# tkkim-robot/safe_control

Hardware: AMD Instinct MI355X
Metric: QP solves/sec (batched agents) (higher is better)
Workload: dtype f64; 1 GPU; 4096-agent batch DynamicUnicycle2D CBF-QP, 8 obstacles each (BASELINE configs[1]); agents_per_gpu=4096, obstacles=8, storage=f32, arithmetic=f64, launch=hipGraph

## Files before the change

### safe_control_amd/csrc/cbf_qp_kernel.hpp

```cpp
#pragma once
#include <hip/hip_runtime.h>

#include <utility>

#include <cstdlib>

#include "sc_qp2.hpp"
#include "sc_group.hpp"

namespace sc {

#ifndef SC_COOP_MAX_AGENTS
#define SC_COOP_MAX_AGENTS 32768
#endif

static inline long long sc_coop_max_agents() {
    static const long long v = [] { const char* e = getenv("SC_COOP_MAX_AGENTS"); return e ? atoll(e) : (long long)SC_COOP_MAX_AGENTS; }();
    return v;
}
static inline bool sc_two_pass() {
    static const bool v = [] { const char* e = getenv("SC_CBFQP_TWO_PASS"); return !(e && e[0] == '0'); }();
    return v;
}
static inline bool sc_force_lds_kernel() {
    static const bool v = [] { const char* e = getenv("SC_FORCE_LDS_KERNEL"); return e && e[0] == '1'; }();
    return v;
}

using as1_void = const __attribute__((address_space(1))) void;
using as3_void = __attribute__((address_space(3))) void;

template <typename TIO, int MODEL>
struct StateRow { TIO v[MODEL == SC_MODEL_QUAD2D ? 5 : 4]; };

template <typename TIO, int MODEL>
__device__ __forceinline__ StateRow<TIO, MODEL> load_state(const TIO* __restrict__ X, long long agent) {
    StateRow<TIO, MODEL> s;
    if constexpr (MODEL == SC_MODEL_QUAD2D) {
        const TIO* r = X + agent * 6;
#pragma unroll
        for (int i = 0; i < 5; ++i) s.v[i] = r[i];
    } else {
        const TIO* r = X + agent * 4;
#pragma unroll
        for (int i = 0; i < 4; ++i) s.v[i] = r[i];
    }
    return s;
}

template <typename TIO, typename TC, int MODEL>
__device__ __forceinline__ Agent<TC> to_agent(const StateRow<TIO, MODEL>& s) {
    if constexpr (MODEL == SC_MODEL_QUAD2D) return make_agent_m<TC, MODEL>(TC(s.v[0]), TC(s.v[1]), TC(s.v[2]), TC(s.v[3]), TC(s.v[4]));
    else return make_agent_m<TC, MODEL>(TC(s.v[0]), TC(s.v[1]), TC(s.v[2]), TC(s.v[3]));
}

template <typename TIO, typename TC, int MODEL>
__device__ __forceinline__ Agent<TC> load_agent(const TIO* __restrict__ X, long long agent) {
    return to_agent<TIO, TC, MODEL>(load_state<TIO, MODEL>(X, agent));
}

template <typename T>
__device__ __forceinline__ void fetch_arg_now(const T& v) { asm volatile("" ::"s"(v)); }

template <typename TIO> struct vec2;
template <> struct vec2<float> { using type = float2; };
template <> struct vec2<double> { using type = double2; };

__device__ __forceinline__ void wave_dma16(const unsigned char* __restrict__ src, unsigned char* lds,
                                           unsigned bytes, int lane) {
    const unsigned n16 = bytes >> 4;
    for (unsigned base = 0; base < n16; base += 64) {
        const unsigned idx = base + lane;
        if (idx < n16) {
            __builtin_amdgcn_global_load_lds((as1_void*)(src + (size_t)idx * 16),
                                             (as3_void*)(lds + (size_t)base * 16), 16, 0, 0);
        }
    }
}

template <typename TIO> struct vec4io;
template <> struct vec4io<float> { using type = float4; static constexpr int N = 4; };
template <> struct vec4io<double> { using type = double2; static constexpr int N = 2; };

#define SC_STATUS_PENDING (-1)
template <typename TIO, typename TC, int KMAX, int MODEL, int PASS = 0>
__global__ __launch_bounds__(256) void cbfqp_reg_kernel(const TIO* __restrict__ obs, const TIO* __restrict__ X,
                                                        const TIO* __restrict__ u_ref, const int* __restrict__ n_obs,
                                                        const long long B, const int K, const int obs_shared,
                                                        TIO* __restrict__ u_out, int* __restrict__ status_out,
                                                        TIO* __restrict__ h_out, const CbfConsts<TC> k) {
    const long long agent = (long long)blockIdx.x * blockDim.x + threadIdx.x;
    const bool active = agent < B;
    const long long ag_i = active ? agent : 0;
    using V2 = typename vec2<TIO>::type;
    using V4 = typename vec4io<TIO>::type;
    constexpr int VN = vec4io<TIO>::N;
    if constexpr (PASS == 2) {
        const bool pending = active && status_out[ag_i] == SC_STATUS_PENDING;
        if (__builtin_amdgcn_ballot_w64(pending) == 0ull) return;
    }

    TIO flat[KMAX * 7];
    const TIO* src = obs + (obs_shared ? 0 : (size_t)ag_i * K * 7);
    if (K == KMAX && ((KMAX * 7) % VN == 0) && ((reinterpret_cast<uintptr_t>(obs) & 15u) == 0) &&
        ((KMAX * 7 * sizeof(TIO)) % 16 == 0)) {
        const V4* s4 = reinterpret_cast<const V4*>(src);
#pragma unroll
        for (int e = 0; e < KMAX * 7 / VN; ++e) {
            const V4 q = s4[e];
            if constexpr (VN == 4) {
                flat[e * 4 + 0] = q.x; flat[e * 4 + 1] = q.y; flat[e * 4 + 2] = q.z; flat[e * 4 + 3] = q.w;
            } else {
                flat[e * 2 + 0] = q.x; flat[e * 2 + 1] = q.y;
            }
        }
    } else {
#pragma unroll
        for (int r = 0; r < KMAX; ++r) {
#pragma unroll
            for (int f = 0; f < 7; ++f) flat[r * 7 + f] = (r < K) ? src[r * 7 + f] : TIO(0);
        }
    }
    const V2 ur = reinterpret_cast<const V2*>(u_ref)[ag_i];
    const StateRow<TIO, MODEL> xs = load_state<TIO, MODEL>(X, ag_i);
    int nk = K;
    if (n_obs) nk = n_obs[ag_i];
    nk = nk < 0 ? 0 : (nk > K ? K : nk);
    if constexpr (PASS == 1) {
        bool other = false;
#pragma unroll
        for (int r = 0; r < KMAX; ++r) other |= (r < nk) && (flat[r * 7 + 6] != TIO(0));
        if (__builtin_amdgcn_ballot_w64(other && active) != 0ull) {
            if (active) status_out[agent] = SC_STATUS_PENDING;
            return;
        }
    }
    const TC ur0 = TC(ur.x), ur1 = TC(ur.y);
    const Agent<TC> ag = to_agent<TIO, TC, MODEL>(xs);

    TC n0[KMAX], n1[KMAX], c[KMAX];
    TIO hv[KMAX];
    bool bad_obs = false;
    TC poison = TC(0);
#pragma unroll
    for (int r = 0; r < KMAX; ++r) {
        TC o[7];
#pragma unroll
        for (int f = 0; f < 7; ++f) o[f] = TC(flat[r * 7 + f]);
        TC h, a0, a1, cc;
        const bool ok = cbf_row<TC, MODEL, true, PASS == 1>(ag, o, k, a0, a1, cc, h);
        const bool used = r < nk;
        bad_obs |= used && !ok;
        a0 = used ? a0 : TC(0); a1 = used ? a1 : TC(0); cc = used ? cc : TC(0);
        normalise_row(a0, a1, cc, poison);
        n0[r] = a0; n1[r] = a1; c[r] = cc;
        hv[r] = used ? TIO(h) : TIO(0);
    }

    TC u0, u1;
    int st = qp2_solve<TC, KMAX>(n0, n1, c, K, ur0, ur1, poison, k, u0, u1);
    if (bad_obs) st = SC_STATUS_BAD_OBSTACLE;
    if (st != SC_STATUS_OPTIMAL) { u0 = num<TC>::nan(); u1 = num<TC>::nan(); }
    if (active) {
        V2 uo; uo.x = TIO(u0); uo.y = TIO(u1);
        reinterpret_cast<V2*>(u_out)[agent] = uo;
        status_out[agent] = st;
        if (h_out) {
            TIO* hp = h_out + agent * K;
            if (K == KMAX && (KMAX % VN == 0) && ((reinterpret_cast<uintptr_t>(h_out) & 15u) == 0)) {
                V4* h4 = reinterpret_cast<V4*>(hp);
#pragma unroll
                for (int e = 0; e < KMAX / VN; ++e) {
                    V4 q;
                    if constexpr (VN == 4) { q.x = hv[e * 4]; q.y = hv[e * 4 + 1]; q.z = hv[e * 4 + 2]; q.w = hv[e * 4 + 3]; }
                    else { q.x = hv[e * 2]; q.y = hv[e * 2 + 1]; }
                    h4[e] = q;
                }
            } else {
#pragma unroll
                for (int r = 0; r < KMAX; ++r) if (r < K) hp[r] = hv[r];
            }
        }
    }
}

template <typename TIO, typename TC, int G, int MODEL>
#ifndef SC_COOP_WAVES
#define SC_COOP_WAVES 1
#endif
__global__ __launch_bounds__(64 * SC_COOP_WAVES) void cbfqp_coop_kernel(const TIO* __restrict__ obs, const TIO* __restrict__ X,
                                                        const TIO* __restrict__ u_ref, const int* __restrict__ n_obs,
                                                        const long long B, const int K, const int obs_shared,
                                                        TIO* __restrict__ u_out, int* __restrict__ status_out,
                                                        TIO* __restrict__ h_out, const CbfConsts<TC> k) {
#ifdef SC_EXP_EMPTY
    return;
#endif
    constexpr int APW = 64 / G;
    const int lane = threadIdx.x & 63;
    const int sub = lane & (G - 1);
    const long long agent = ((long long)blockIdx.x * SC_COOP_WAVES + (threadIdx.x >> 6)) * APW + lane / G;
    const bool active = agent < B;
    const long long ag_i = active ? agent : 0;
    using V2 = typename vec2<TIO>::type;
#ifdef SC_EXP_ARGS
    if (active && sub == 0)
        status_out[agent] = (int)((reinterpret_cast<uintptr_t>(obs) ^ reinterpret_cast<uintptr_t>(X) ^ reinterpret_cast<uintptr_t>(u_ref) ^
                                   reinterpret_cast<uintptr_t>(n_obs) ^ reinterpret_cast<uintptr_t>(u_out) ^ reinterpret_cast<uintptr_t>(h_out)) >> 4) + K + obs_shared;
    return;
#endif

    TIO orow[7];
    const bool has_row = sub < K;
    const TIO* src = obs + (obs_shared ? 0 : (size_t)ag_i * K * 7) + (has_row ? sub * 7 : 0);
#pragma unroll
    for (int f = 0; f < 7; ++f) orow[f] = src[f];
    const V2 ur = reinterpret_cast<const V2*>(u_ref)[ag_i];
    const StateRow<TIO, MODEL> xs = load_state<TIO, MODEL>(X, ag_i);
    int nk = K;
    if (n_obs) nk = n_obs[ag_i];
    nk = nk < 0 ? 0 : (nk > K ? K : nk);
    fetch_arg_now(status_out); fetch_arg_now(h_out);
    fetch_arg_now(k.R); fetch_arg_now(k.g1); fetch_arg_now(k.g2);
    fetch_arg_now(k.lo0); fetch_arg_now(k.hi0); fetch_arg_now(k.lo1); fetch_arg_now(k.hi1); fetch_arg_now(k.hard);
#ifdef SC_EXP_LOADS
    if (active) {
        if (sub == 0) {
            V2 uo; uo.x = ur.x + xs.v[0] + xs.v[1]; uo.y = ur.y + xs.v[2] + xs.v[3];
            reinterpret_cast<V2*>(u_out)[agent] = uo;
            status_out[agent] = nk;
        }
        if (h_out && has_row) h_out[agent * K + sub] = orow[0] + orow[1] + orow[2] + orow[3] + orow[4] + orow[5] + orow[6];
    }
    return;
#endif
    const TC ur0 = TC(ur.x), ur1 = TC(ur.y);
    const Agent<TC> ag = to_agent<TIO, TC, MODEL>(xs);

    TC o[7];
#pragma unroll
    for (int f = 0; f < 7; ++f) o[f] = TC(orow[f]);
    TC h, a0, a1, cc;
#ifndef SC_EXP_NOROW
    const bool ok = cbf_row<TC, MODEL, false>(ag, o, k, a0, a1, cc, h);
#else
    const bool ok = true; a0 = o[0] - ag.x; a1 = o[1] - ag.y; cc = o[2]; h = o[3];
#endif
    const bool used = sub < nk;
    const bool bad_mine = used && !ok;
    a0 = used ? a0 : TC(0); a1 = used ? a1 : TC(0); cc = used ? cc : TC(0);
    if (active && h_out && has_row) h_out[agent * K + sub] = used ? TIO(h) : TIO(0);
    TC poison = TC(0);
    normalise_row(a0, a1, cc, poison);

    QpState<TC> S;
    qp_begin(S, ur0, ur1, k);
#ifndef SC_EXP_NOWALK
#ifndef SC_COOP_OLD_WALK
    if constexpr (G == 8) coop_solve_all8<TC>(S, K, sub, lane, a0, a1, cc, k);
    else if constexpr (G == 16) coop_solve_all16<TC>(S, K, sub, lane, a0, a1, cc, k);
    else
#endif
    coop_walk_violated<TC, G>(S, K, sub, lane, a0, a1, cc, k);
#endif
    qp_finish_box(S, k);
    TC worst = qp_row_margin(num<TC>::inf(), a0, a1, cc, S.u0, S.u1, poison);
    const bool nan_mine = !(poison == poison);
    worst = nan_mine ? -num<TC>::inf() : worst;
    if constexpr (G == 8) worst = min8_raw(worst);
    else if constexpr (G == 16) worst = min16_raw(worst);
    else worst = group_min<TC, G>(worst);
    const unsigned long long bad_mask = __builtin_amdgcn_ballot_w64(bad_mine);
    const bool bad_any = ((bad_mask >> (lane & ~(G - 1))) & (G == 64 ? ~0ull : ((1ull << G) - 1ull))) != 0ull;
    int st = qp_status(S, worst, TC(0), k);
    if (bad_any) st = SC_STATUS_BAD_OBSTACLE;
    TC u0 = S.u0, u1 = S.u1;
    if (st != SC_STATUS_OPTIMAL) { u0 = num<TC>::nan(); u1 = num<TC>::nan(); }
    if (active) {
        if (sub == 0) {
            V2 uo; uo.x = TIO(u0); uo.y = TIO(u1);
            reinterpret_cast<V2*>(u_out)[agent] = uo;
            status_out[agent] = st;
        }
    }
}

typedef double sc_d8 __attribute__((ext_vector_type(8)));
struct Coop8Consts {
    sc_d8 t0;
    sc_d8 t1;
    sc_d8 k0;
    sc_d8 k1;
    int hard;
    unsigned B;
};

__device__ __forceinline__ void normalise_row_as_generic(double& n0, double& n1, double& c, double& poison) {
    const double nn = __builtin_fma(n1, n1, n0 * n0);
    poison += 0.0 * (nn + c);
    const double inv = nn > 0.0 ? rsqrt_(nn) : 1.0;
    n0 *= inv; n1 *= inv; c *= inv;
}

template <typename TIO, bool FULL, bool HAS_H>
__global__ __launch_bounds__(64) void cbfqp_coop8_du_kernel(const TIO* __restrict__ obs, const TIO* __restrict__ X,
                                                            const TIO* __restrict__ u_ref, TIO* __restrict__ u_out,
                                                            TIO* __restrict__ h_out, int* __restrict__ status_out,
                                                            const Coop8Consts c) {
#ifdef SC_EXP_EMPTY
    return;
#endif
    using TC = double;
    using V2 = typename vec2<TIO>::type;
    const unsigned lane = threadIdx.x;
    const unsigned sub = lane & 7u;
    const unsigned slot = blockIdx.x * 64u + lane;
    const unsigned agent = slot >> 3;
    bool active = true;
    if constexpr (!FULL) active = agent < c.B;
    const unsigned row_i = active ? slot : sub;
    const unsigned ag_i = row_i >> 3;

    struct { TIO v[7]; } orow;
    __builtin_memcpy(&orow, obs + row_i * 7u, sizeof(orow));
    const V2 ur = reinterpret_cast<const V2*>(u_ref)[ag_i];
    const StateRow<TIO, SC_MODEL_DYNAMIC_UNICYCLE2D> xs = load_state<TIO, SC_MODEL_DYNAMIC_UNICYCLE2D>(X, ag_i);
    fetch_arg_now(c.t0); fetch_arg_now(c.t1); fetch_arg_now(c.k0); fetch_arg_now(c.k1); fetch_arg_now(c.hard);

    SinCosTab sc;
    sc.two_over_pi = c.t0[0]; sc.pio2_1 = c.t0[1]; sc.pio2_2 = c.t0[2]; sc.pio2_3 = c.t0[3];
    sc.s[0] = c.t0[4]; sc.s[1] = c.t0[5]; sc.s[2] = c.t0[6]; sc.s[3] = c.t0[7]; sc.s[4] = c.t1[0]; sc.s[5] = c.t1[1];
#pragma unroll
    for (int i = 0; i < 6; ++i) sc.c[i] = c.t1[2 + i];
    CbfConsts<TC> k;
    k.R = c.k0[0]; k.a1 = TC(0); k.a2 = TC(0); k.g1 = c.k0[1]; k.g2 = c.k0[2]; k.inv_dt = c.k0[3]; k.inv_dt2 = c.k0[4];
    k.lo0 = c.k0[5]; k.hi0 = c.k0[6]; k.lo1 = c.k0[7]; k.hi1 = c.k1[0]; k.inv_Lr = TC(0); k.inv_mass = TC(1); k.hard = c.hard;
    BoxTol<TC> bt;
    bt.lo0 = c.k1[1]; bt.hi0 = c.k1[2]; bt.lo1 = c.k1[3]; bt.hi1 = c.k1[4];

    const TC ur0 = TC(ur.x), ur1 = TC(ur.y);
    Agent<TC> ag;
    ag.x = TC(xs.v[0]); ag.y = TC(xs.v[1]); ag.th = TC(xs.v[2]); ag.v = TC(xs.v[3]);
    sincos_tab_sfma(ag.th, sc, &ag.s, &ag.c);
    ag.f0 = ag.v * ag.c;
    ag.f1 = ag.v * ag.s;

    TC o[7];
#pragma unroll
    for (int f = 0; f < 7; ++f) o[f] = TC(orow.v[f]);
    TC h, a0, a1, cc;
    const bool ok = cbf_row<TC, SC_MODEL_DYNAMIC_UNICYCLE2D, false>(ag, o, k, a0, a1, cc, h);
    const bool bad_mine = !ok;
    if constexpr (HAS_H) {
        if (active) h_out[slot] = TIO(h);
    }
    TC poison = TC(0);
    normalise_row_as_generic(a0, a1, cc, poison);

    QpState<TC> S;
    qp_begin_raw(S, ur0, ur1, k);
    coop_solve_all8_full<TC>(S, (int)sub, (int)lane, a0, a1, cc, k, bt);
    qp_finish_box_raw(S, k);
    TC worst = qp_row_margin_raw(a0, a1, cc, S.u0, S.u1, poison);
    const bool nan_mine = !(poison == poison);
    worst = nan_mine ? -num<TC>::inf() : worst;
    worst = min8_raw(worst);
    int st = qp_status(S, worst, TC(0), k);
    if (__builtin_amdgcn_ballot_w64(bad_mine) != 0ull) {
        asm volatile("");
        const unsigned long long bad_mask = __builtin_amdgcn_ballot_w64(bad_mine);
        const bool bad_any = ((bad_mask >> (lane & ~7u)) & 0xffull) != 0ull;
        if (bad_any) st = SC_STATUS_BAD_OBSTACLE;
    }
    TC u0 = S.u0, u1 = S.u1;
    if (st != SC_STATUS_OPTIMAL) { u0 = num<TC>::nan(); u1 = num<TC>::nan(); }
    if (active && sub == 0) {
        V2 uo; uo.x = TIO(u0); uo.y = TIO(u1);
        reinterpret_cast<V2*>(u_out)[agent] = uo;
        status_out[agent] = st;
    }
}

#if defined(SC_EXP_GRID) && !defined(SC_EXP_EMPTY)
#error "SC_EXP_GRID needs SC_EXP_EMPTY: a kernel with a body would run past the batch"
#endif
static inline unsigned coop_grid(unsigned nblk) {
#ifdef SC_EXP_GRID
    return SC_EXP_GRID;
#else
    return nblk;
#endif
}

static inline bool sc_cbfqp_generic() {
    static const bool v = [] { const char* e = getenv("SC_CBFQP_GENERIC"); return e && e[0] == '1'; }();
    return v;
}

static inline double sc_quieted(double x) {
    if (x != x) {
        unsigned long long b;
        __builtin_memcpy(&b, &x, sizeof(b));
        b |= 0x0008000000000000ull;
        __builtin_memcpy(&x, &b, sizeof(b));
    }
    return x;
}

template <typename TIO>
static hipError_t launch_coop8_du(const sc_cbfqp_params& p, long long B, const void* X, const void* u_ref, const void* obs,
                                  void* u_out, int* status, void* h_out, hipStream_t stream) {
    const CbfConsts<double> k = make_consts<double>(p);
    const BoxTol<double> bt = box_tol(k);
    const SinCosTab t = make_sincos_tab();
    Coop8Consts c;
    c.t0 = sc_d8{t.two_over_pi, t.pio2_1, t.pio2_2, t.pio2_3, t.s[0], t.s[1], t.s[2], t.s[3]};
    c.t1 = sc_d8{t.s[4], t.s[5], t.c[0], t.c[1], t.c[2], t.c[3], t.c[4], t.c[5]};
    c.k0 = sc_d8{k.R, k.g1, k.g2, k.inv_dt, k.inv_dt2, sc_quieted(k.lo0), sc_quieted(k.hi0), sc_quieted(k.lo1)};
    c.k1 = sc_d8{sc_quieted(k.hi1), bt.lo0, bt.hi0, bt.lo1, bt.hi1, 0.0, 0.0, 0.0};
    c.hard = k.hard;
    c.B = (unsigned)B;
    const dim3 grid(coop_grid((unsigned)((B + 7) / 8))), block(64);
#define SC_GO(FULL, HAS_H)                                                                                             \
    hipLaunchKernelGGL((cbfqp_coop8_du_kernel<TIO, FULL, HAS_H>), grid, block, 0, stream, (const TIO*)obs, (const TIO*)X, \
                       (const TIO*)u_ref, (TIO*)u_out, (TIO*)h_out, status, c)
    if (B % 8 == 0) { if (h_out) SC_GO(true, true); else SC_GO(true, false); }
    else { if (h_out) SC_GO(false, true); else SC_GO(false, false); }
#undef SC_GO
    return hipGetLastError();
}

template <typename TIO, typename TC, int G, int MODEL>
static hipError_t launch_coop(const sc_cbfqp_params& p, long long B, int K, const void* X, const void* u_ref,
                              const void* obs, const int* n_obs, void* u_out, int* status, void* h_out,
                              hipStream_t stream) {
    if constexpr (G == 8 && MODEL == SC_MODEL_DYNAMIC_UNICYCLE2D && sizeof(TC) == 8 && SC_COOP_WAVES == 1) {
        if (K == 8 && n_obs == nullptr && p.obs_shared == 0 && B >= 1 && B <= sc_coop_max_agents() &&
            B * 8 * 7 * (long long)sizeof(TIO) <= 0x7fffffffLL && !sc_cbfqp_generic())
            return launch_coop8_du<TIO>(p, B, X, u_ref, obs, u_out, status, h_out, stream);
    }
    constexpr int APW = 64 / G;
    const unsigned nblk = coop_grid((unsigned)((B + APW * SC_COOP_WAVES - 1) / (APW * SC_COOP_WAVES)));
    const CbfConsts<TC> k = make_consts<TC>(p);
    hipLaunchKernelGGL((cbfqp_coop_kernel<TIO, TC, G, MODEL>), dim3(nblk), dim3(64 * SC_COOP_WAVES), 0, stream,
                       (const TIO*)obs, (const TIO*)X, (const TIO*)u_ref, n_obs, B, K, (int)p.obs_shared,
                       (TIO*)u_out, status, (TIO*)h_out, k);
    return hipGetLastError();
}

template <typename TIO, typename TC, int KMAX, int MODEL>
__global__ __launch_bounds__(64) void cbfqp_kernel(const TIO* __restrict__ obs, const TIO* __restrict__ X,
                                                   const TIO* __restrict__ u_ref, const int* __restrict__ n_obs,
                                                   const long long B, const int K, const int obs_shared,
                                                   TIO* __restrict__ u_out, int* __restrict__ status_out,
                                                   TIO* __restrict__ h_out, const CbfConsts<TC> k) {
    extern __shared__ __attribute__((aligned(16))) unsigned char smem[];
    TIO* lobs = reinterpret_cast<TIO*>(smem);

    const int lane = threadIdx.x;
    const long long first = (long long)blockIdx.x * 64;
    const long long agent = first + lane;
    const int nag = (int)((B - first) < 64 ? (B - first) : 64);
    const bool active = lane < nag;
    const int row_elems = K * 7;

    if (obs_shared) {
        for (int e = lane; e < row_elems; e += 64) lobs[e] = obs[e];
    } else {
        const TIO* src = obs + (size_t)first * row_elems;
        const unsigned bytes = (unsigned)nag * row_elems * sizeof(TIO);
        if ((bytes & 15u) == 0 && ((reinterpret_cast<uintptr_t>(src) & 15u) == 0)) {
            wave_dma16(reinterpret_cast<const unsigned char*>(src), smem, bytes, lane);
        } else {
            const int total = nag * row_elems;
            for (int e = lane; e < total; e += 64) lobs[e] = src[e];
        }
    }

    using V2 = typename vec2<TIO>::type;
    const long long ag_i = active ? agent : 0;
    const V2 ur = reinterpret_cast<const V2*>(u_ref)[ag_i];
    const StateRow<TIO, MODEL> xs = load_state<TIO, MODEL>(X, ag_i);
    int nk = K;
    if (n_obs) nk = n_obs[ag_i];
    nk = !active ? K : (nk < 0 ? 0 : (nk > K ? K : nk));
    const TC ur0 = active ? TC(ur.x) : TC(0), ur1 = active ? TC(ur.y) : TC(0);
    const Agent<TC> ag = to_agent<TIO, TC, MODEL>(xs);

    asm volatile("s_waitcnt vmcnt(0)" ::: "memory");
    __syncthreads();

    const size_t stage_bytes = ((obs_shared ? (size_t)row_elems : (size_t)64 * row_elems) * sizeof(TIO) + 15) & ~(size_t)15;
    TC* rows = reinterpret_cast<TC*>(smem + stage_bytes);
    TIO* hl = reinterpret_cast<TIO*>(rows + (size_t)K * 3 * 64);
    const TIO* mine = lobs + (obs_shared ? 0 : lane * row_elems);
    int period = 32;
    while (((K * (32 / period)) & 31) != 0 && period > 1) period >>= 1;
    const int rot = obs_shared ? 0 : (lane / period) % K;
    bool bad_obs = false;
    TC poison = TC(0);
#pragma nounroll
    for (int r = 0; r < K; ++r) {
        int ro = r + rot;
        ro = ro >= K ? ro - K : ro;
        TC o[7];
#pragma unroll
        for (int f = 0; f < 7; ++f) o[f] = TC(mine[ro * 7 + f]);
        TC h, a0, a1, cc;
        const bool ok = cbf_row<TC, MODEL>(ag, o, k, a0, a1, cc, h);
        const bool used = ro < nk;
        bad_obs |= used && !ok;
        a0 = used ? a0 : TC(0); a1 = used ? a1 : TC(0); cc = used ? cc : TC(0);
        normalise_row(a0, a1, cc, poison);
        rows[(ro * 3 + 0) * 64 + lane] = a0;
        rows[(ro * 3 + 1) * 64 + lane] = a1;
        rows[(ro * 3 + 2) * 64 + lane] = cc;
        if constexpr (KMAX > 0) {
            hl[ro * 64 + lane] = used ? TIO(h) : TIO(0);
        } else {
            if (active && h_out) h_out[agent * K + ro] = used ? TIO(h) : TIO(0);
        }
    }

    TC u0, u1;
    int st;
    if constexpr (KMAX > 0) {
        TC n0[KMAX], n1[KMAX], c[KMAX];
#pragma unroll
        for (int j = 0; j < KMAX; ++j) {
            const bool in = j < K;
            n0[j] = in ? rows[(j * 3 + 0) * 64 + lane] : TC(0);
            n1[j] = in ? rows[(j * 3 + 1) * 64 + lane] : TC(0);
            c[j] = in ? rows[(j * 3 + 2) * 64 + lane] : TC(0);
        }
        st = qp2_solve<TC, KMAX>(n0, n1, c, K, ur0, ur1, poison, k, u0, u1);
    } else {
        st = qp2_solve_lds<TC>(rows, lane, K, ur0, ur1, poison, k, u0, u1);
    }

    if (bad_obs) st = SC_STATUS_BAD_OBSTACLE;
    if (st != SC_STATUS_OPTIMAL) { u0 = num<TC>::nan(); u1 = num<TC>::nan(); }

    if (active) {
        V2 uo; uo.x = TIO(u0); uo.y = TIO(u1);
        reinterpret_cast<V2*>(u_out)[agent] = uo;
        status_out[agent] = st;
        if constexpr (KMAX > 0) {
            if (h_out) {
                TIO* hp = h_out + agent * K;
                if (K == KMAX) {
                    TIO hv[KMAX];
#pragma unroll
                    for (int r = 0; r < KMAX; ++r) hv[r] = hl[r * 64 + lane];
#pragma unroll
                    for (int r = 0; r < KMAX; ++r) hp[r] = hv[r];
                } else {
                    for (int r = 0; r < K; ++r) hp[r] = hl[r * 64 + lane];
                }
            }
        }
    }
}

template <typename TIO, typename TC, int KMAX, int MODEL>
static hipError_t launch_one(const sc_cbfqp_params& p, long long B, int K, const void* X, const void* u_ref,
                             const void* obs, const int* n_obs, void* u_out, int* status, void* h_out,
                             hipStream_t stream) {
    if constexpr (KMAX > 0) {
        if (B <= sc_coop_max_agents())
            return launch_coop<TIO, TC, 8, MODEL>(p, B, K, X, u_ref, obs, n_obs, u_out, status, h_out, stream);
        const unsigned threads = 256;
        const unsigned nblk = (unsigned)((B + threads - 1) / threads);
        const CbfConsts<TC> k = make_consts<TC>(p);
        if constexpr (MODEL == SC_MODEL_DYNAMIC_UNICYCLE2D && sizeof(TC) == 8) {
            if (sc_two_pass() && B >= (1 << 18)) {
                hipLaunchKernelGGL((cbfqp_reg_kernel<TIO, TC, KMAX, MODEL, 1>), dim3(nblk), dim3(threads), 0, stream,
                                   (const TIO*)obs, (const TIO*)X, (const TIO*)u_ref, n_obs, B, K, (int)p.obs_shared,
                                   (TIO*)u_out, status, (TIO*)h_out, k);
                hipError_t e = hipGetLastError();
                if (e != hipSuccess) return e;
                hipLaunchKernelGGL((cbfqp_reg_kernel<TIO, TC, KMAX, MODEL, 2>), dim3(nblk), dim3(threads), 0, stream,
                                   (const TIO*)obs, (const TIO*)X, (const TIO*)u_ref, n_obs, B, K, (int)p.obs_shared,
                                   (TIO*)u_out, status, (TIO*)h_out, k);
                return hipGetLastError();
            }
        }
        hipLaunchKernelGGL((cbfqp_reg_kernel<TIO, TC, KMAX, MODEL>), dim3(nblk), dim3(threads), 0, stream,
                           (const TIO*)obs, (const TIO*)X, (const TIO*)u_ref, n_obs, B, K, (int)p.obs_shared,
                           (TIO*)u_out, status, (TIO*)h_out, k);
        return hipGetLastError();
    } else {
// ... 62 lines not shown
```

### safe_control_amd/csrc/sc_group.hpp

```cpp
#pragma once
#include <hip/hip_runtime.h>

#include <utility>

#include "sc_qp2.hpp"

namespace sc {

template <int CTRL>
__device__ __forceinline__ float dpp_mov(float v) {
    return __int_as_float(__builtin_amdgcn_update_dpp(0, __float_as_int(v), CTRL, 0xf, 0xf, true));
}
template <int CTRL>
__device__ __forceinline__ double dpp_mov(double v) {
    const int lo = __builtin_amdgcn_update_dpp(0, __double2loint(v), CTRL, 0xf, 0xf, true);
    const int hi = __builtin_amdgcn_update_dpp(0, __double2hiint(v), CTRL, 0xf, 0xf, true);
    return __hiloint2double(hi, lo);
}
template <typename T, int G, int I>
__device__ __forceinline__ T group_bcast(T v, int sub) {
    if constexpr (G == 8) {
        const T q = dpp_mov<(I & 3) * 0x55>(v);
        const T m = dpp_mov<0x141>(q);
        return ((sub >> 2) == (I >> 2)) ? q : m;
// ... 70 lines not shown
        last = has ? istar : K;
    }
}

template <typename T, int X>
__device__ __forceinline__ T group_xor8(T v, T mirrored) {
    if constexpr (X == 1) return dpp_mov<0xB1>(v);
    else if constexpr (X == 2) return dpp_mov<0x4E>(v);
    else if constexpr (X == 3) return dpp_mov<0x1B>(v);
    else if constexpr (X == 4) return dpp_mov<0x1B>(mirrored);
    else if constexpr (X == 5) return dpp_mov<0x4E>(mirrored);
    else if constexpr (X == 6) return dpp_mov<0xB1>(mirrored);
    else return mirrored;
}
__device__ __forceinline__ float min_raw(float a, float b) { float r; asm("v_min_f32 %0, %1, %2" : "=v"(r) : "v"(a), "v"(b)); return r; }
__device__ __forceinline__ float max_raw(float a, float b) { float r; asm("v_max_f32 %0, %1, %2" : "=v"(r) : "v"(a), "v"(b)); return r; }
__device__ __forceinline__ double min_raw(double a, double b) { double r; asm("v_min_f64 %0, %1, %2" : "=v"(r) : "v"(a), "v"(b)); return r; }
__device__ __forceinline__ double max_raw(double a, double b) { double r; asm("v_max_f64 %0, %1, %2" : "=v"(r) : "v"(a), "v"(b)); return r; }
__device__ __forceinline__ float max_neg_raw(float a, float b) { float r; asm("v_max_f32 %0, %1, -%2" : "=v"(r) : "v"(a), "v"(b)); return r; }
__device__ __forceinline__ double max_neg_raw(double a, double b) { double r; asm("v_max_f64 %0, %1, -%2" : "=v"(r) : "v"(a), "v"(b)); return r; }
__device__ __forceinline__ float max_abs_one_raw(float a) { float r; asm("v_max_f32 %0, |%1|, 1.0" : "=v"(r) : "v"(a)); return r; }
__device__ __forceinline__ double max_abs_one_raw(double a) { double r; asm("v_max_f64 %0, |%1|, 1.0" : "=v"(r) : "v"(a)); return r; }
__device__ __forceinline__ float keep_or_nan(bool keep, float v) { return keep ? v : __int_as_float(0x7fc00000); }
__device__ __forceinline__ double keep_or_nan(bool keep, double v) {
    return __hiloint2double(keep ? __double2hiint(v) : 0x7ff80000, __double2loint(v));
}
template <typename T>
__device__ __forceinline__ T min8_raw(T v) {
    v = min_raw(v, dpp_mov<0xB1>(v)); v = min_raw(v, dpp_mov<0x4E>(v)); v = min_raw(v, dpp_mov<0x141>(v));
    return v;
}
template <typename T>
__device__ __forceinline__ T min16_raw(T v) { v = min8_raw(v); return min_raw(v, dpp_mov<0x140>(v)); }
template <int CTRL>
__device__ __forceinline__ int or_dpp(int v) { return v | __builtin_amdgcn_update_dpp(0, v, CTRL, 0xf, 0xf, true); }
template <int G>
__device__ __forceinline__ int group_or_bits(int v) {
    v = or_dpp<0xB1>(v); v = or_dpp<0x4E>(v); v = or_dpp<0x141>(v);
    if constexpr (G == 16) v = or_dpp<0x140>(v);
    return v;
}
template <int G>
__device__ __forceinline__ float group_pick(bool mine, float v) { return __int_as_float(group_or_bits<G>(mine ? __float_as_int(v) : 0)); }
template <int G>
__device__ __forceinline__ double group_pick(bool mine, double v) {
    const int lo = group_or_bits<G>(mine ? __double2loint(v) : 0), hi = group_or_bits<G>(mine ? __double2hiint(v) : 0);
    return __hiloint2double(hi, lo);
}

template <typename T>
__device__ __forceinline__ void clip_row_coop(LineQP<T>& L, bool& dead, T g0, T g1, T gc) {
    const T a = g0 * L.d0 + g1 * L.d1;
    const T r = g0 * L.p0 + (g1 * L.p1 + gc);
    const bool pos = a > num<T>::eps_par();
    const bool neg = !(a >= -num<T>::eps_par());
    const bool par_viol = r < -num<T>::tol_feas() * max_abs_one_raw(gc);
    const T q = r * rcp_(fabs_(a));
    dead |= !pos && !neg && par_viol;
    L.lo = max_neg_raw(L.lo, keep_or_nan(pos, q));
    L.hi = min_raw(L.hi, keep_or_nan(neg, q));
}

template <int G>
__device__ __forceinline__ bool group_first(unsigned long long m, int lane, int sub, bool& has) {
    const unsigned bits = (unsigned)(m >> (lane & ~(G - 1))) & ((1u << G) - 1u);
    has = bits != 0u;
    return sub == __builtin_ctz(bits | (1u << G));
}

template <typename TC, int... Xs>
__device__ __forceinline__ void clip_partners8(LineQP<TC>& L, bool& dead, TC a0, TC a1, TC cc, std::integer_sequence<int, Xs...>) {
    const TC m0 = dpp_mov<0x141>(a0), m1 = dpp_mov<0x141>(a1), mc = dpp_mov<0x141>(cc);
    (clip_row_coop(L, dead, group_xor8<TC, Xs + 1>(a0, m0), group_xor8<TC, Xs + 1>(a1, m1), group_xor8<TC, Xs + 1>(cc, mc)), ...);
}
template <typename TC, int G>
__device__ __forceinline__ void coop_pick_winner(QpState<TC>& S, const LineQP<TC>& L, bool ok, int sub, int lane) {
    const TC inf = num<TC>::inf();
    TC t = fmin_(fmax_(TC(0), L.lo), L.hi);
    const bool inverted = L.lo > L.hi;
    t = inverted ? TC(0.5) * (L.lo + L.hi) : t;
    const bool empty = L.lo > L.hi + num<TC>::tol_feas() * fmax_(TC(1), fmax_(fabs_(L.lo), fabs_(L.hi)));
    const TC v0 = L.p0 + t * L.d0, v1 = L.p1 + t * L.d1;
    const TC e0 = v0 - S.ur0, e1 = v1 - S.ur1;
    TC cost = e0 * e0 + e1 * e1;
    cost = (ok && !empty && (cost == cost)) ? cost : inf;
    TC best;
    if constexpr (G == 8) best = min8_raw(cost); else best = min16_raw(cost);
    bool has;
    const bool mine = group_first<G>(__builtin_amdgcn_ballot_w64((cost == best) && (best < inf)), lane, sub, has);
    const TC s0 = group_pick<G>(mine, v0), s1 = group_pick<G>(mine, v1);
    S.u0 = has ? s0 : S.u0;
    S.u1 = has ? s1 : S.u1;
}
template <typename TC>
__device__ __forceinline__ void coop_solve_all8(QpState<TC>& S, int K, int sub, int lane, TC a0, TC a1, TC cc,
                                                const CbfConsts<TC>& k) {
    const bool testable = (sub < K) && !((a0 == TC(0)) && (a1 == TC(0)));
    LineQP<TC> L;
    const bool viol = qp_row_violated(S, a0, a1, cc, L, k) && testable;
    if (__builtin_amdgcn_ballot_w64(viol) == 0ull) return;
    clip_box(L, k);
    bool dead = false;
    clip_partners8(L, dead, a0, a1, cc, std::make_integer_sequence<int, 7>{});
    coop_pick_winner<TC, 8>(S, L, viol && !dead, sub, lane);
}

template <typename T>
struct BoxTol { T lo0, hi0, lo1, hi1; };
template <typename T>
__host__ __device__ inline BoxTol<T> box_tol(const CbfConsts<T>& k) {
    const T tol = sizeof(T) == 8 ? T(1e-9) : T(1e-5f);
    BoxTol<T> b;
    b.lo0 = k.lo0 - tol; b.hi0 = k.hi0 + tol; b.lo1 = k.lo1 - tol; b.hi1 = k.hi1 + tol;
    return b;
}
template <typename T>
__device__ __forceinline__ void clip_box_tol(LineQP<T>& L, const CbfConsts<T>& k, const BoxTol<T>& bt) {
    const T inf = num<T>::inf();
    {
        const T r = rcp_(L.d0);
        const T t1 = (k.lo0 - L.p0) * r, t2 = (k.hi0 - L.p0) * r;
        const bool flat = L.d0 == T(0);
        const bool inside = (L.p0 >= bt.lo0) && (L.p0 <= bt.hi0);
        const T lo = flat ? (inside ? -inf : inf) : fmin_(t1, t2);
        const T hi = flat ? inf : fmax_(t1, t2);
        L.lo = lo; L.hi = hi;
    }
    {
        const T r = rcp_(L.d1);
        const T t1 = (k.lo1 - L.p1) * r, t2 = (k.hi1 - L.p1) * r;
        const bool flat = L.d1 == T(0);
        const bool inside = (L.p1 >= bt.lo1) && (L.p1 <= bt.hi1);
        const T lo = flat ? (inside ? -inf : inf) : fmin_(t1, t2);
        const T hi = flat ? inf : fmax_(t1, t2);
        L.lo = fmax_(L.lo, lo); L.hi = fmin_(L.hi, hi);
    }
}

__device__ __forceinline__ double max_raw_s(double a, double b) { double r; asm("v_max_f64 %0, %1, %2" : "=v"(r) : "v"(a), "s"(b)); return r; }
__device__ __forceinline__ double min_raw_s(double a, double b) { double r; asm("v_min_f64 %0, %1, %2" : "=v"(r) : "v"(a), "s"(b)); return r; }
__device__ __forceinline__ double max_zero_raw(double a) { double r; asm("v_max_f64 %0, %1, 0" : "=v"(r) : "v"(a)); return r; }
__device__ __forceinline__ double max_one_raw(double a) { double r; asm("v_max_f64 %0, %1, 1.0" : "=v"(r) : "v"(a)); return r; }
__device__ __forceinline__ double max_abs_abs_raw(double a, double b) { double r; asm("v_max_f64 %0, |%1|, |%2|" : "=v"(r) : "v"(a), "v"(b)); return r; }

__device__ __forceinline__ void qp_begin_raw(QpState<double>& S, double ur0, double ur1, const CbfConsts<double>& k) {
    S.ur0 = ur0; S.ur1 = ur1;
    S.u0 = min_raw_s(max_raw_s(ur0, k.lo0), k.hi0);
    S.u1 = min_raw_s(max_raw_s(ur1, k.lo1), k.hi1);
}
__device__ __forceinline__ void qp_finish_box_raw(QpState<double>& S, const CbfConsts<double>& k) {
    S.u0 = min_raw_s(max_raw_s(S.u0, k.lo0), k.hi0);
    S.u1 = min_raw_s(max_raw_s(S.u1, k.lo1), k.hi1);
}
__device__ __forceinline__ double qp_row_margin_raw(double a0, double a1, double ci, double u0, double u1, double& poison) {
    const double s = a0 * u0 + (a1 * u1 + ci);
    const double m = s + num<double>::tol_feas() * max_abs_one_raw(ci);
    poison += 0.0 * s;
    return fmin_(num<double>::inf(), m);
}

template <typename T>
__device__ __forceinline__ void clip_box_tol_lazy(LineQP<T>& L, const CbfConsts<T>& k, const BoxTol<T>& bt) {
    const T r0 = rcp_(L.d0), r1 = rcp_(L.d1);
    const T t1 = (k.lo0 - L.p0) * r0, t2 = (k.hi0 - L.p0) * r0;
    const T t3 = (k.lo1 - L.p1) * r1, t4 = (k.hi1 - L.p1) * r1;
    const bool flat = (L.d0 == T(0)) || (L.d1 == T(0));
    L.lo = fmax_(fmin_(t1, t2), fmin_(t3, t4));
    L.hi = fmin_(fmax_(t1, t2), fmax_(t3, t4));
    if (__builtin_amdgcn_ballot_w64(flat) != 0ull) clip_box_tol(L, k, bt);
}

template <typename T>
__device__ __forceinline__ void clip_row_coop_lazy(LineQP<T>& L, bool& anypar, T g0, T g1, T gc) {
    const T a = g0 * L.d0 + g1 * L.d1;
    const T r = g0 * L.p0 + (g1 * L.p1 + gc);
    const bool pos = a > num<T>::eps_par();
    const bool neg = !(a >= -num<T>::eps_par());
    const T q = r * rcp_(fabs_(a));
    anypar |= !pos && !neg;
    L.lo = max_neg_raw(L.lo, keep_or_nan(pos, q));
    L.hi = min_raw(L.hi, keep_or_nan(neg, q));
}
template <typename TC, int... Xs>
__device__ __forceinline__ void clip_partners8_lazy(LineQP<TC>& L, bool& anypar, TC a0, TC a1, TC cc, std::integer_sequence<int, Xs...>) {
    const TC m0 = dpp_mov<0x141>(a0), m1 = dpp_mov<0x141>(a1), mc = dpp_mov<0x141>(cc);
    (clip_row_coop_lazy(L, anypar, group_xor8<TC, Xs + 1>(a0, m0), group_xor8<TC, Xs + 1>(a1, m1), group_xor8<TC, Xs + 1>(cc, mc)), ...);
}
template <typename T>
__device__ __forceinline__ bool row_dead_coop(const LineQP<T>& L, T g0, T g1, T gc) {
    const T a = g0 * L.d0 + g1 * L.d1;
    const T r = g0 * L.p0 + (g1 * L.p1 + gc);
    const bool pos = a > num<T>::eps_par();
    const bool neg = !(a >= -num<T>::eps_par());
    const bool par_viol = r < -num<T>::tol_feas() * max_abs_one_raw(gc);
    return !pos && !neg && par_viol;
}
template <typename TC>
__device__ __forceinline__ bool partners8_dead(const LineQP<TC>& L, TC a0, TC a1, TC cc) {
    bool dead = false;
#pragma nounroll
    for (int x = 1; x < 8; ++x) dead |= row_dead_coop(L, __shfl_xor(a0, x, 8), __shfl_xor(a1, x, 8), __shfl_xor(cc, x, 8));
    return dead;
}

__device__ __forceinline__ void coop_pick_winner8_raw(QpState<double>& S, const LineQP<double>& L, bool ok, int sub, int lane) {
    using TC = double;
    const TC inf = num<TC>::inf();
    TC t = min_raw(max_zero_raw(L.lo), L.hi);
    const bool inverted = L.lo > L.hi;
    t = inverted ? TC(0.5) * (L.lo + L.hi) : t;
    const bool empty = L.lo > L.hi + num<TC>::tol_feas() * max_one_raw(max_abs_abs_raw(L.lo, L.hi));
    const TC v0 = L.p0 + t * L.d0, v1 = L.p1 + t * L.d1;
    const TC e0 = v0 - S.ur0, e1 = v1 - S.ur1;
    TC cost = e0 * e0 + e1 * e1;
    cost = (ok && !empty && (cost == cost)) ? cost : inf;
    const TC best = min8_raw(cost);
    bool has;
    const bool mine = group_first<8>(__builtin_amdgcn_ballot_w64((cost == best) && (best < inf)), lane, sub, has);
    const TC s0 = group_pick<8>(mine, v0), s1 = group_pick<8>(mine, v1);
    S.u0 = has ? s0 : S.u0;
    S.u1 = has ? s1 : S.u1;
}

template <typename TC>
__device__ __forceinline__ void coop_solve_all8_full(QpState<TC>& S, int sub, int lane, TC a0, TC a1, TC cc,
                                                     const CbfConsts<TC>& k, const BoxTol<TC>& bt) {
    const bool testable = !((a0 == TC(0)) && (a1 == TC(0)));
    LineQP<TC> L;
    const bool viol = qp_row_violated(S, a0, a1, cc, L, k) && testable;
    if (__builtin_amdgcn_ballot_w64(viol) == 0ull) return;
    clip_box_tol_lazy(L, k, bt);
    bool anypar = false;
    clip_partners8_lazy(L, anypar, a0, a1, cc, std::make_integer_sequence<int, 7>{});
    bool dead = false;
    if (__builtin_amdgcn_ballot_w64(anypar) != 0ull)
        dead = partners8_dead(L, a0, a1, cc);
    coop_pick_winner8_raw(S, L, viol && !dead, sub, lane);
}

template <typename TC, int... Rs>
__device__ __forceinline__ void clip_partners16(LineQP<TC>& L, bool& dead, TC a0, TC a1, TC cc, std::integer_sequence<int, Rs...>) {
    (clip_row_coop(L, dead, dpp_mov<0x121 + Rs>(a0), dpp_mov<0x121 + Rs>(a1), dpp_mov<0x121 + Rs>(cc)), ...);
}
template <typename TC>
__device__ __forceinline__ void coop_solve_all16(QpState<TC>& S, int K, int sub, int lane, TC a0, TC a1, TC cc,
                                                 const CbfConsts<TC>& k) {
    const bool testable = (sub < K) && !((a0 == TC(0)) && (a1 == TC(0)));
    LineQP<TC> L;
    const bool viol = qp_row_violated(S, a0, a1, cc, L, k) && testable;
    if (__builtin_amdgcn_ballot_w64(viol) == 0ull) return;
    clip_box(L, k);
    bool dead = false;
    clip_partners16(L, dead, a0, a1, cc, std::make_integer_sequence<int, 15>{});
    coop_pick_winner<TC, 16>(S, L, viol && !dead, sub, lane);
}

}
```

Before: 1.626 billion solves/s.

## Micro-tune coop8 DU kernel: template hard flag, literal consts, cheaper parallel check

The hard flag becomes a template parameter, and the feasibility tolerance, parallel epsilon and infinity literals are now passed in kernel-argument constant vectors instead of being materialised in code. The per-partner parallel test is replaced by a running min of |a| checked once with a ballot. The rsqrt guard is made wave-uniform-lazy, and address math uses 24-bit multiplies and byte offsets. The intent is to cut VALU instructions, SGPR/VGPR pressure and literal moves in this already tight kernel. The cost is an extra template instantiation and a new limit on B*8 that sends larger batches to the fallback path.

```diff
diff --git a/safe_control_amd/csrc/cbf_qp_kernel.hpp b/safe_control_amd/csrc/cbf_qp_kernel.hpp
--- a/safe_control_amd/csrc/cbf_qp_kernel.hpp
+++ b/safe_control_amd/csrc/cbf_qp_kernel.hpp
@@ -1,6 +1,7 @@
 #pragma once
 #include <hip/hip_runtime.h>
 
+#include <type_traits>
 #include <utility>
 
 #include <cstdlib>
@@ -291,18 +292,27 @@
     sc_d8 t1;
     sc_d8 k0;
     sc_d8 k1;
-    int hard;
     unsigned B;
 };
 
 __device__ __forceinline__ void normalise_row_as_generic(double& n0, double& n1, double& c, double& poison) {
     const double nn = __builtin_fma(n1, n1, n0 * n0);
     poison += 0.0 * (nn + c);
-    const double inv = nn > 0.0 ? rsqrt_(nn) : 1.0;
+    double inv = rsqrt_(nn);
+    if (__builtin_amdgcn_ballot_w64(!(nn > 0.0)) != 0ull) {
+        asm volatile("");
+        inv = nn > 0.0 ? inv : 1.0;
+    }
     n0 *= inv; n1 *= inv; c *= inv;
 }
 
-template <typename TIO, bool FULL, bool HAS_H>
+template <typename T>
+__device__ __forceinline__ T* at_byte(T* base, unsigned off) {
+    using C = typename std::conditional<std::is_const<T>::value, const char, char>::type;
+    return reinterpret_cast<T*>(reinterpret_cast<C*>(base) + off);
+}
+
+template <typename TIO, bool FULL, bool HAS_H, bool HARD>
 __global__ __launch_bounds__(64) void cbfqp_coop8_du_kernel(const TIO* __restrict__ obs, const TIO* __restrict__ X,
                                                             const TIO* __restrict__ u_ref, TIO* __restrict__ u_out,
                                                             TIO* __restrict__ h_out, int* __restrict__ status_out,
@@ -319,13 +329,14 @@
     bool active = true;
     if constexpr (!FULL) active = agent < c.B;
     const unsigned row_i = active ? slot : sub;
-    const unsigned ag_i = row_i >> 3;
+    const unsigned ag8 = row_i & ~7u;
 
     struct { TIO v[7]; } orow;
-    __builtin_memcpy(&orow, obs + row_i * 7u, sizeof(orow));
-    const V2 ur = reinterpret_cast<const V2*>(u_ref)[ag_i];
-    const StateRow<TIO, SC_MODEL_DYNAMIC_UNICYCLE2D> xs = load_state<TIO, SC_MODEL_DYNAMIC_UNICYCLE2D>(X, ag_i);
-    fetch_arg_now(c.t0); fetch_arg_now(c.t1); fetch_arg_now(c.k0); fetch_arg_now(c.k1); fetch_arg_now(c.hard);
+    __builtin_memcpy(&orow, at_byte(obs, __umul24(row_i, 7u * (unsigned)sizeof(TIO))), sizeof(orow));
+    const V2 ur = *reinterpret_cast<const V2*>(at_byte(u_ref, ag8 * (unsigned)(sizeof(V2) / 8)));
+    StateRow<TIO, SC_MODEL_DYNAMIC_UNICYCLE2D> xs;
+    __builtin_memcpy(&xs, at_byte(X, ag8 * (unsigned)(sizeof(xs) / 8)), sizeof(xs));
+    fetch_arg_now(c.t0); fetch_arg_now(c.t1); fetch_arg_now(c.k0); fetch_arg_now(c.k1);
 
     SinCosTab sc;
     sc.two_over_pi = c.t0[0]; sc.pio2_1 = c.t0[1]; sc.pio2_2 = c.t0[2]; sc.pio2_3 = c.t0[3];
@@ -334,9 +345,11 @@
     for (int i = 0; i < 6; ++i) sc.c[i] = c.t1[2 + i];
     CbfConsts<TC> k;
     k.R = c.k0[0]; k.a1 = TC(0); k.a2 = TC(0); k.g1 = c.k0[1]; k.g2 = c.k0[2]; k.inv_dt = c.k0[3]; k.inv_dt2 = c.k0[4];
-    k.lo0 = c.k0[5]; k.hi0 = c.k0[6]; k.lo1 = c.k0[7]; k.hi1 = c.k1[0]; k.inv_Lr = TC(0); k.inv_mass = TC(1); k.hard = c.hard;
+    k.lo0 = c.k0[5]; k.hi0 = c.k0[6]; k.lo1 = c.k0[7]; k.hi1 = c.k1[0]; k.inv_Lr = TC(0); k.inv_mass = TC(1); k.hard = HARD;
     BoxTol<TC> bt;
     bt.lo0 = c.k1[1]; bt.hi0 = c.k1[2]; bt.lo1 = c.k1[3]; bt.hi1 = c.k1[4];
+    SolveLit<TC> lit;
+    lit.tol_feas = c.k1[5]; lit.eps_par = c.k1[6]; lit.inf = c.k1[7];
 
     const TC ur0 = TC(ur.x), ur1 = TC(ur.y);
     Agent<TC> ag;
@@ -352,20 +365,20 @@
     const bool ok = cbf_row<TC, SC_MODEL_DYNAMIC_UNICYCLE2D, false>(ag, o, k, a0, a1, cc, h);
     const bool bad_mine = !ok;
     if constexpr (HAS_H) {
-        if (active) h_out[slot] = TIO(h);
+        if (active) *at_byte(h_out, slot * (unsigned)sizeof(TIO)) = TIO(h);
     }
     TC poison = TC(0);
     normalise_row_as_generic(a0, a1, cc, poison);
 
     QpState<TC> S;
     qp_begin_raw(S, ur0, ur1, k);
-    coop_solve_all8_full<TC>(S, (int)sub, (int)lane, a0, a1, cc, k, bt);
+    coop_solve_all8_full<TC>(S, (int)sub, (int)lane, a0, a1, cc, k, bt, lit);
     qp_finish_box_raw(S, k);
-    TC worst = qp_row_margin_raw(a0, a1, cc, S.u0, S.u1, poison);
+    TC worst = qp_row_margin_raw(a0, a1, cc, S.u0, S.u1, poison, lit);
     const bool nan_mine = !(poison == poison);
     worst = nan_mine ? -num<TC>::inf() : worst;
     worst = min8_raw(worst);
-    int st = qp_status(S, worst, TC(0), k);
+    int st = qp_status_lit(S, worst, TC(0), k, lit);
     if (__builtin_amdgcn_ballot_w64(bad_mine) != 0ull) {
         asm volatile("");
         const unsigned long long bad_mask = __builtin_amdgcn_ballot_w64(bad_mine);
@@ -417,15 +430,16 @@
     c.t0 = sc_d8{t.two_over_pi, t.pio2_1, t.pio2_2, t.pio2_3, t.s[0], t.s[1], t.s[2], t.s[3]};
     c.t1 = sc_d8{t.s[4], t.s[5], t.c[0], t.c[1], t.c[2], t.c[3], t.c[4], t.c[5]};
     c.k0 = sc_d8{k.R, k.g1, k.g2, k.inv_dt, k.inv_dt2, sc_quieted(k.lo0), sc_quieted(k.hi0), sc_quieted(k.lo1)};
-    c.k1 = sc_d8{sc_quieted(k.hi1), bt.lo0, bt.hi0, bt.lo1, bt.hi1, 0.0, 0.0, 0.0};
-    c.hard = k.hard;
+    c.k1 = sc_d8{sc_quieted(k.hi1), bt.lo0, bt.hi0, bt.lo1, bt.hi1, 1e-9, 1e-12, __builtin_huge_val()};
     c.B = (unsigned)B;
     const dim3 grid(coop_grid((unsigned)((B + 7) / 8))), block(64);
-#define SC_GO(FULL, HAS_H)                                                                                             \
-    hipLaunchKernelGGL((cbfqp_coop8_du_kernel<TIO, FULL, HAS_H>), grid, block, 0, stream, (const TIO*)obs, (const TIO*)X, \
+#define SC_GO(FULL, HAS_H, HARD)                                                                                             \
+    hipLaunchKernelGGL((cbfqp_coop8_du_kernel<TIO, FULL, HAS_H, HARD>), grid, block, 0, stream, (const TIO*)obs, (const TIO*)X, \
                        (const TIO*)u_ref, (TIO*)u_out, (TIO*)h_out, status, c)
-    if (B % 8 == 0) { if (h_out) SC_GO(true, true); else SC_GO(true, false); }
-    else { if (h_out) SC_GO(false, true); else SC_GO(false, false); }
+#define SC_GO_H(FULL, HAS_H) do { if (k.hard) SC_GO(FULL, HAS_H, true); else SC_GO(FULL, HAS_H, false); } while (0)
+    if (B % 8 == 0) { if (h_out) SC_GO_H(true, true); else SC_GO_H(true, false); }
+    else { if (h_out) SC_GO_H(false, true); else SC_GO_H(false, false); }
+#undef SC_GO_H
 #undef SC_GO
     return hipGetLastError();
 }
@@ -436,7 +450,7 @@
                               hipStream_t stream) {
     if constexpr (G == 8 && MODEL == SC_MODEL_DYNAMIC_UNICYCLE2D && sizeof(TC) == 8 && SC_COOP_WAVES == 1) {
         if (K == 8 && n_obs == nullptr && p.obs_shared == 0 && B >= 1 && B <= sc_coop_max_agents() &&
-            B * 8 * 7 * (long long)sizeof(TIO) <= 0x7fffffffLL && !sc_cbfqp_generic())
+            B * 8 * 7 * (long long)sizeof(TIO) <= 0x7fffffffLL && B * 8 <= 0xffffffLL && !sc_cbfqp_generic())
             return launch_coop8_du<TIO>(p, B, X, u_ref, obs, u_out, status, h_out, stream);
     }
     constexpr int APW = 64 / G;
diff --git a/safe_control_amd/csrc/sc_group.hpp b/safe_control_amd/csrc/sc_group.hpp
--- a/safe_control_amd/csrc/sc_group.hpp
+++ b/safe_control_amd/csrc/sc_group.hpp
@@ -246,11 +246,21 @@
     S.u0 = min_raw_s(max_raw_s(S.u0, k.lo0), k.hi0);
     S.u1 = min_raw_s(max_raw_s(S.u1, k.lo1), k.hi1);
 }
-__device__ __forceinline__ double qp_row_margin_raw(double a0, double a1, double ci, double u0, double u1, double& poison) {
+template <typename T>
+struct SolveLit { T tol_feas, eps_par, inf; };
+
+__device__ __forceinline__ double qp_row_margin_raw(double a0, double a1, double ci, double u0, double u1, double& poison,
+                                                    const SolveLit<double>& lit) {
     const double s = a0 * u0 + (a1 * u1 + ci);
-    const double m = s + num<double>::tol_feas() * max_abs_one_raw(ci);
+    const double m = s + lit.tol_feas * max_abs_one_raw(ci);
     poison += 0.0 * s;
-    return fmin_(num<double>::inf(), m);
+    return fmin_(lit.inf, m);
+}
+__device__ __forceinline__ int qp_status_lit(const QpState<double>& S, double worst, double poison, const CbfConsts<double>& k,
+                                             const SolveLit<double>& lit) {
+    const bool finite = (poison == poison) && (fabs_(S.ur0 + S.ur1) < lit.inf);
+    const bool box_ok = (k.lo0 <= k.hi0) && (k.lo1 <= k.hi1);
+    return (!(worst >= 0.0) || !finite || !box_ok) ? SC_STATUS_INFEASIBLE : SC_STATUS_OPTIMAL;
 }
 
 template <typename T>
@@ -264,21 +274,34 @@
     if (__builtin_amdgcn_ballot_w64(flat) != 0ull) clip_box_tol(L, k, bt);
 }
 
-template <typename T>
-__device__ __forceinline__ void clip_row_coop_lazy(LineQP<T>& L, bool& anypar, T g0, T g1, T gc) {
-    const T a = g0 * L.d0 + g1 * L.d1;
-    const T r = g0 * L.p0 + (g1 * L.p1 + gc);
-    const bool pos = a > num<T>::eps_par();
-    const bool neg = !(a >= -num<T>::eps_par());
-    const T q = r * rcp_(fabs_(a));
-    anypar |= !pos && !neg;
+__device__ __forceinline__ double min_abs_abs_raw(double a, double b) { double r; asm("v_min_f64 %0, |%1|, |%2|" : "=v"(r) : "v"(a), "v"(b)); return r; }
+__device__ __forceinline__ double min_abs_raw(double a, double b) { double r; asm("v_min_f64 %0, %1, |%2|" : "=v"(r) : "v"(a), "v"(b)); return r; }
+__device__ __forceinline__ double clip_row_coop_lazy(LineQP<double>& L, double eps, double g0, double g1, double gc) {
+    const double a = g0 * L.d0 + g1 * L.d1;
+    const double r = g0 * L.p0 + (g1 * L.p1 + gc);
+    const bool pos = a > eps;
+    const bool neg = !(a >= -eps);
+    const double q = r * rcp_(fabs_(a));
     L.lo = max_neg_raw(L.lo, keep_or_nan(pos, q));
     L.hi = min_raw(L.hi, keep_or_nan(neg, q));
-}
-template <typename TC, int... Xs>
-__device__ __forceinline__ void clip_partners8_lazy(LineQP<TC>& L, bool& anypar, TC a0, TC a1, TC cc, std::integer_sequence<int, Xs...>) {
-    const TC m0 = dpp_mov<0x141>(a0), m1 = dpp_mov<0x141>(a1), mc = dpp_mov<0x141>(cc);
-    (clip_row_coop_lazy(L, anypar, group_xor8<TC, Xs + 1>(a0, m0), group_xor8<TC, Xs + 1>(a1, m1), group_xor8<TC, Xs + 1>(cc, mc)), ...);
+    return a;
+}
+template <int X>
+__device__ __forceinline__ double clip_partner8_lazy(LineQP<double>& L, double eps, double a0, double a1, double cc, double m0, double m1,
+                                                     double mc) {
+    return clip_row_coop_lazy(L, eps, group_xor8<double, X>(a0, m0), group_xor8<double, X>(a1, m1), group_xor8<double, X>(cc, mc));
+}
+__device__ __forceinline__ double clip_partners8_lazy(LineQP<double>& L, double eps, double a0, double a1, double cc) {
+    const double m0 = dpp_mov<0x141>(a0), m1 = dpp_mov<0x141>(a1), mc = dpp_mov<0x141>(cc);
+    const double x1 = clip_partner8_lazy<1>(L, eps, a0, a1, cc, m0, m1, mc);
+    const double x2 = clip_partner8_lazy<2>(L, eps, a0, a1, cc, m0, m1, mc);
+    double amin = min_abs_abs_raw(x1, x2);
+    amin = min_abs_raw(amin, clip_partner8_lazy<3>(L, eps, a0, a1, cc, m0, m1, mc));
+    amin = min_abs_raw(amin, clip_partner8_lazy<4>(L, eps, a0, a1, cc, m0, m1, mc));
+    amin = min_abs_raw(amin, clip_partner8_lazy<5>(L, eps, a0, a1, cc, m0, m1, mc));
+    amin = min_abs_raw(amin, clip_partner8_lazy<6>(L, eps, a0, a1, cc, m0, m1, mc));
+    amin = min_abs_raw(amin, clip_partner8_lazy<7>(L, eps, a0, a1, cc, m0, m1, mc));
+    return amin;
 }
 template <typename T>
 __device__ __forceinline__ bool row_dead_coop(const LineQP<T>& L, T g0, T g1, T gc) {
@@ -297,20 +320,21 @@
     return dead;
 }
 
-__device__ __forceinline__ void coop_pick_winner8_raw(QpState<double>& S, const LineQP<double>& L, bool ok, int sub, int lane) {
+__device__ __forceinline__ void coop_pick_winner8_raw(QpState<double>& S, const LineQP<double>& L, bool ok, int sub, int lane,
+                                                      const SolveLit<double>& lit) {
     using TC = double;
     const TC inf = num<TC>::inf();
     TC t = min_raw(max_zero_raw(L.lo), L.hi);
     const bool inverted = L.lo > L.hi;
     t = inverted ? TC(0.5) * (L.lo + L.hi) : t;
-    const bool empty = L.lo > L.hi + num<TC>::tol_feas() * max_one_raw(max_abs_abs_raw(L.lo, L.hi));
+    const bool empty = L.lo > L.hi + lit.tol_feas * max_one_raw(max_abs_abs_raw(L.lo, L.hi));
     const TC v0 = L.p0 + t * L.d0, v1 = L.p1 + t * L.d1;
     const TC e0 = v0 - S.ur0, e1 = v1 - S.ur1;
     TC cost = e0 * e0 + e1 * e1;
     cost = (ok && !empty && (cost == cost)) ? cost : inf;
     const TC best = min8_raw(cost);
     bool has;
-    const bool mine = group_first<8>(__builtin_amdgcn_ballot_w64((cost == best) && (best < inf)), lane, sub, has);
+    const bool mine = group_first<8>(__builtin_amdgcn_ballot_w64((cost == best) && (best < lit.inf)), lane, sub, has);
     const TC s0 = group_pick<8>(mine, v0), s1 = group_pick<8>(mine, v1);
     S.u0 = has ? s0 : S.u0;
     S.u1 = has ? s1 : S.u1;
@@ -318,18 +342,17 @@
 
 template <typename TC>
 __device__ __forceinline__ void coop_solve_all8_full(QpState<TC>& S, int sub, int lane, TC a0, TC a1, TC cc,
-                                                     const CbfConsts<TC>& k, const BoxTol<TC>& bt) {
+                                                     const CbfConsts<TC>& k, const BoxTol<TC>& bt, const SolveLit<TC>& lit) {
     const bool testable = !((a0 == TC(0)) && (a1 == TC(0)));
     LineQP<TC> L;
     const bool viol = qp_row_violated(S, a0, a1, cc, L, k) && testable;
     if (__builtin_amdgcn_ballot_w64(viol) == 0ull) return;
     clip_box_tol_lazy(L, k, bt);
-    bool anypar = false;
-    clip_partners8_lazy(L, anypar, a0, a1, cc, std::make_integer_sequence<int, 7>{});
+    const TC amin = clip_partners8_lazy(L, lit.eps_par, a0, a1, cc);
     bool dead = false;
-    if (__builtin_amdgcn_ballot_w64(anypar) != 0ull)
+    if (__builtin_amdgcn_ballot_w64(amin <= lit.eps_par) != 0ull)
         dead = partners8_dead(L, a0, a1, cc);
-    coop_pick_winner8_raw(S, L, viol && !dead, sub, lane);
+    coop_pick_winner8_raw(S, L, viol && !dead, sub, lane, lit);
 }
 
 template <typename TC, int... Rs>
```

Result: faster. 1.676 billion solves/s, median of 6 (+3.1%).
